# dfm/george

Measured on NVIDIA H100. Metric: gp.compute+log_likelihood N-points/sec, higher is better.
Workload: dtype f64

## Files before the change

george_b200/csrc/hodlr_leaf.cuh:

```cuda
#pragma once

#include "gemm_dmma.cuh"
#include "hodlr_kernels.cuh"

namespace bgp {

constexpr int LF_THREADS = 256;
constexpr int LF_NB = 32;
constexpr int LF_MAX_LEAF = 768;

__host__ __device__ inline int lf_panel_ld(int max_m) { return ((max_m + 15) / 16) * 16 + 4; }

template <int SHAPE>
__global__ void __launch_bounds__(LF_THREADS, 2) leaf_factor_kernel(const DevProgram* __restrict__ gprog,
                                                                    const double* __restrict__ x,
                                                                    const double* __restrict__ diag,
                                                                    const LeafDesc* __restrict__ leaves,
                                                                    double* __restrict__ Lbuf,
                                                                    double* __restrict__ leaf_logdet, int ldp) {
  extern __shared__ __align__(16) double lf_smem[];
  double* pn = lf_smem;
  double* dall = lf_smem + LF_NB * ldp;
  DevProgram* P = reinterpret_cast<DevProgram*>(lf_smem + (LF_NB + 1) * ldp);
  __shared__ double red[32];
  __shared__ double dinv[LF_NB];
  if constexpr (SHAPE == BGP_SHAPE_GENERIC) stage_program(P, gprog);
  __syncthreads();
  const auto fn = ShapeEval<SHAPE>::make(P, gprog);
  const LeafDesc lf = leaves[blockIdx.x];
  const int m = lf.size, nd = gprog->ndim;
  double* A = Lbuf + lf.off;
  const double* xs = x + (int64_t)lf.start * nd;
  const int lane = threadIdx.x & 31, warp = threadIdx.x >> 5;

  double logdet = 0.0;
  for (int k0 = 0; k0 < m; k0 += LF_NB) {
    const int nb = min(LF_NB, m - k0), rem = m - k0;
    for (int t = threadIdx.x; t < nb * rem; t += LF_THREADS) {
      const int c = t / rem, i = t - c * rem;
      if (i >= c) {
        double v = fn(xs + (int64_t)(k0 + i) * nd, xs + (int64_t)(k0 + c) * nd);
        if (i == c) v += diag[lf.start + k0 + i];
        pn[c * ldp + i] = v;
      }
    }
    __syncthreads();
    if (k0 > 0) {
      const int lr = lane >> 2, lc = lane & 3;
      const int n_tiles = (rem + 15) / 16;
      bool bok[4];
#pragma unroll
      for (int b = 0; b < 4; ++b) bok[b] = b * 8 + lr < nb;
      for (int t = warp; t < n_tiles; t += LF_THREADS / 32) {
        const int r0 = t * 16;
        bool aok[2];
#pragma unroll
        for (int a = 0; a < 2; ++a) aok[a] = r0 + a * 8 + lr < rem;
        double acc[2][4][2];
#pragma unroll
        for (int a = 0; a < 2; ++a)
#pragma unroll
          for (int b = 0; b < 4; ++b) { acc[a][b][0] = 0.0; acc[a][b][1] = 0.0; }
#pragma unroll 4
        for (int q0 = 0; q0 < k0; q0 += 4) {
          const int q = q0 + lc;
          const double* Lq = A + (int64_t)q * m + k0;
          const double dq = dall[q];
          double af[2], bf[4];
#pragma unroll
          for (int a = 0; a < 2; ++a) af[a] = aok[a] ? Lq[r0 + a * 8 + lr] : 0.0;
#pragma unroll
          for (int b = 0; b < 4; ++b) bf[b] = bok[b] ? Lq[b * 8 + lr] * dq : 0.0;
#pragma unroll
          for (int a = 0; a < 2; ++a)
#pragma unroll
            for (int b = 0; b < 4; ++b) dmma884(acc[a][b][0], acc[a][b][1], af[a], bf[b]);
        }
#pragma unroll
        for (int a = 0; a < 2; ++a) {
          const int i = r0 + a * 8 + lr;
#pragma unroll
          for (int b = 0; b < 4; ++b)
#pragma unroll
            for (int e = 0; e < 2; ++e) {
              const int c = b * 8 + 2 * lc + e;
              if (i < rem && c < nb && i >= c) pn[c * ldp + i] -= acc[a][b][e];
            }
        }
      }
      __syncthreads();
    }
    if (warp == 0) {
      double w[LF_NB];
#pragma unroll
      for (int j = 0; j < LF_NB; ++j) w[j] = (j <= lane && lane < nb) ? pn[j * ldp + lane] : 0.0;
#pragma unroll
      for (int k = 0; k < LF_NB; ++k) {
        if (k < nb) {
          const double d = __shfl_sync(0xffffffffu, w[k], k);
          const double l = (lane > k && lane < nb) ? w[k] / d : 0.0;
          if (lane > k) w[k] = l;
          const double ld = l * d;
#pragma unroll
          for (int j = k + 1; j < LF_NB; ++j) {
            const double lj = __shfl_sync(0xffffffffu, l, j);
            if (j <= lane) w[j] -= ld * lj;
          }
        }
      }
      if (lane < nb) {
        double* col = A + (int64_t)k0 * m + k0 + lane;
        double d = 0.0;
#pragma unroll
        for (int j = 0; j < LF_NB; ++j) {
          if (j < lane) { pn[j * ldp + lane] = w[j]; col[(int64_t)j * m] = w[j]; }
          if (j == lane) d = w[j];
        }
        col[(int64_t)lane * m] = d;
        dall[k0 + lane] = d;
        dinv[lane] = 1.0 / d;
        logdet += log(fabs(d));
      }
    }
    __syncthreads();
    const volatile double* l11 = pn;
    for (int i = LF_NB + threadIdx.x; i < rem; i += LF_THREADS) {
      double w[LF_NB];
#pragma unroll
      for (int j = 0; j < LF_NB; ++j) w[j] = pn[j * ldp + i];
#pragma unroll
      for (int j = 0; j < LF_NB; ++j) {
        double s = w[j];
#pragma unroll
        for (int q = 0; q < j; ++q) s -= w[q] * l11[q * ldp + j];
        w[j] = s;
      }
      double* row = A + (int64_t)k0 * m + k0 + i;
#pragma unroll
      for (int j = 0; j < LF_NB; ++j) row[(int64_t)j * m] = w[j] * dinv[j];
    }
    __syncthreads();
  }
  logdet = block_sum(logdet, red);
  if (threadIdx.x == 0) leaf_logdet[blockIdx.x] = logdet;
}

__host__ inline size_t lf_smem_bytes(int shape, int max_m) {
  return sizeof(double) * (size_t)(LF_NB + 1) * lf_panel_ld(max_m) + (shape == BGP_SHAPE_GENERIC ? sizeof(DevProgram) : 0);
}

template <int SHAPE>
inline void leaf_factor_launch_shape(int n_leaves, int max_m, cudaStream_t s, const DevProgram* prog, const double* x,
                                     const double* diag, const LeafDesc* leaves, double* L, double* leaf_logdet) {
  const size_t smem = lf_smem_bytes(SHAPE, max_m);
  cudaFuncSetAttribute(leaf_factor_kernel<SHAPE>, cudaFuncAttributeMaxDynamicSharedMemorySize, (int)smem);
  leaf_factor_kernel<SHAPE><<<n_leaves, LF_THREADS, smem, s>>>(prog, x, diag, leaves, L, leaf_logdet, lf_panel_ld(max_m));
}

inline void leaf_factor_launch(int shape, int n_leaves, int max_m, cudaStream_t s, const DevProgram* prog,
                               const double* x, const double* diag, const LeafDesc* leaves, double* L,
                               double* leaf_logdet) {
  BGP_SHAPE_SWITCH(shape, (leaf_factor_launch_shape<SHAPE>(n_leaves, max_m, s, prog, x, diag, leaves, L, leaf_logdet)));
}

}
```

Measured before the change: 21.53 million.

## Invert diagonal block and apply panel solve via DMMA in leaf factorization

Replaces the per-row scalar triangular solve for the below-diagonal panel with an explicit inverse of the unit-lower 32x32 diagonal block, computed by warp shuffles, followed by a DMMA tensor-core GEMM. It also rewrites the diagonal LDL factorization as a shifting-register loop using a shared column buffer, adds a 4-way ILP kernel evaluation for non-generic shapes, and raises the unroll on the trailing update. Optional clock64 phase timing instrumentation is added under a compile flag. The goal is to move the serial-heavy panel solve onto tensor cores. In exchange it adds static shared memory, which can affect occupancy, and an explicit inverse is numerically less stable than forward substitution.

Result: faster. 22.81 million, median of 6 (+5.9%).

```diff
diff --git a/george_b200/csrc/hodlr_leaf.cuh b/george_b200/csrc/hodlr_leaf.cuh
--- a/george_b200/csrc/hodlr_leaf.cuh
+++ b/george_b200/csrc/hodlr_leaf.cuh
@@ -8,8 +8,44 @@
 constexpr int LF_THREADS = 256;
 constexpr int LF_NB = 32;
 constexpr int LF_MAX_LEAF = 768;
-
-__host__ __device__ inline int lf_panel_ld(int max_m) { return ((max_m + 15) / 16) * 16 + 4; }
+constexpr int LF_LDT = LF_NB + 4;
+
+__host__ __device__ constexpr int lf_panel_ld(int max_m) { return ((max_m + 15) / 16) * 16 + 4; }
+static_assert((LF_THREADS / 32) * 4 == LF_NB, "step (3b) gives each warp four columns of L11^-1");
+
+#ifdef BGP_LF_PHASE_TIMING
+__device__ unsigned long long lf_phase_cycles[5];
+__device__ unsigned int lf_phase_ctas;
+__device__ inline void lf_phase_report(const long long* ph, long long t_begin) {
+  if (threadIdx.x != 0) return;
+  for (int p = 0; p < 4; ++p) atomicAdd(&lf_phase_cycles[p], (unsigned long long)ph[p]);
+  atomicAdd(&lf_phase_cycles[4], (unsigned long long)(clock64() - t_begin));
+  __threadfence();
+  if (atomicAdd(&lf_phase_ctas, 1u) == gridDim.x - 1) {
+    const double c = 1.0 / gridDim.x;
+    printf("leaf_factor cycles per CTA (%u CTAs): build %.0f update %.0f diagonal %.0f below %.0f total %.0f\n",
+           gridDim.x, lf_phase_cycles[0] * c, lf_phase_cycles[1] * c, lf_phase_cycles[2] * c, lf_phase_cycles[3] * c,
+           lf_phase_cycles[4] * c);
+    for (int p = 0; p < 5; ++p) lf_phase_cycles[p] = 0;
+    lf_phase_ctas = 0;
+  }
+}
+#define LF_TIMER_INIT                      \
+  long long lf_ph[4] = {0, 0, 0, 0};       \
+  const long long lf_t0 = clock64();       \
+  long long lf_t = lf_t0;
+#define LF_STAMP(p)                          \
+  if (threadIdx.x == 0) {                    \
+    const long long t1_ = clock64();         \
+    lf_ph[p] += t1_ - lf_t;                  \
+    lf_t = t1_;                              \
+  }
+#define LF_TIMER_REPORT lf_phase_report(lf_ph, lf_t0);
+#else
+#define LF_TIMER_INIT
+#define LF_STAMP(p)
+#define LF_TIMER_REPORT
+#endif
 
 template <int SHAPE>
 __global__ void __launch_bounds__(LF_THREADS, 2) leaf_factor_kernel(const DevProgram* __restrict__ gprog,
@@ -23,7 +59,8 @@
   double* dall = lf_smem + LF_NB * ldp;
   DevProgram* P = reinterpret_cast<DevProgram*>(lf_smem + (LF_NB + 1) * ldp);
   __shared__ double red[32];
-  __shared__ double dinv[LF_NB];
+  __shared__ __align__(16) double tm[LF_NB * LF_LDT];
+  __shared__ double colb[2 * LF_NB];
   if constexpr (SHAPE == BGP_SHAPE_GENERIC) stage_program(P, gprog);
   __syncthreads();
   const auto fn = ShapeEval<SHAPE>::make(P, gprog);
@@ -32,19 +69,31 @@
   double* A = Lbuf + lf.off;
   const double* xs = x + (int64_t)lf.start * nd;
   const int lane = threadIdx.x & 31, warp = threadIdx.x >> 5;
+  constexpr int ilp = SHAPE == BGP_SHAPE_GENERIC ? 1 : 4;
 
   double logdet = 0.0;
+  LF_TIMER_INIT
   for (int k0 = 0; k0 < m; k0 += LF_NB) {
     const int nb = min(LF_NB, m - k0), rem = m - k0;
-    for (int t = threadIdx.x; t < nb * rem; t += LF_THREADS) {
-      const int c = t / rem, i = t - c * rem;
-      if (i >= c) {
-        double v = fn(xs + (int64_t)(k0 + i) * nd, xs + (int64_t)(k0 + c) * nd);
-        if (i == c) v += diag[lf.start + k0 + i];
-        pn[c * ldp + i] = v;
+    const bool below = rem > LF_NB;
+    for (int t0 = threadIdx.x; t0 < nb * rem; t0 += LF_THREADS * ilp) {
+      double v[ilp];
+      int ci[ilp], ii[ilp];
+#pragma unroll
+      for (int u = 0; u < ilp; ++u) {
+        const int t = min(t0 + u * LF_THREADS, nb * rem - 1);
+        ci[u] = t / rem;
+        ii[u] = t - ci[u] * rem;
+        v[u] = fn(xs + (int64_t)(k0 + ii[u]) * nd, xs + (int64_t)(k0 + ci[u]) * nd);
+      }
+#pragma unroll
+      for (int u = 0; u < ilp; ++u) {
+        const int c = ci[u], i = ii[u];
+        if (t0 + u * LF_THREADS < nb * rem && i >= c) pn[c * ldp + i] = i == c ? v[u] + diag[lf.start + k0 + i] : v[u];
       }
     }
     __syncthreads();
+    LF_STAMP(0)
     if (k0 > 0) {
       const int lr = lane >> 2, lc = lane & 3;
       const int n_tiles = (rem + 15) / 16;
@@ -61,7 +110,7 @@
         for (int a = 0; a < 2; ++a)
 #pragma unroll
           for (int b = 0; b < 4; ++b) { acc[a][b][0] = 0.0; acc[a][b][1] = 0.0; }
-#pragma unroll 4
+#pragma unroll 8
         for (int q0 = 0; q0 < k0; q0 += 4) {
           const int q = q0 + lc;
           const double* Lq = A + (int64_t)q * m + k0;
@@ -89,65 +138,105 @@
         }
       }
       __syncthreads();
+      LF_STAMP(1)
     }
     if (warp == 0) {
+      const int i = lane;
       double w[LF_NB];
 #pragma unroll
-      for (int j = 0; j < LF_NB; ++j) w[j] = (j <= lane && lane < nb) ? pn[j * ldp + lane] : 0.0;
-#pragma unroll
-      for (int k = 0; k < LF_NB; ++k) {
-        if (k < nb) {
-          const double d = __shfl_sync(0xffffffffu, w[k], k);
-          const double l = (lane > k && lane < nb) ? w[k] / d : 0.0;
-          if (lane > k) w[k] = l;
-          const double ld = l * d;
-#pragma unroll
-          for (int j = k + 1; j < LF_NB; ++j) {
-            const double lj = __shfl_sync(0xffffffffu, l, j);
-            if (j <= lane) w[j] -= ld * lj;
+      for (int j = 0; j < LF_NB; ++j) w[j] = (j <= i && i < nb) ? pn[j * ldp + i] : 0.0;
+      double dmine = 1.0;
+      for (int k = 0; k < nb; ++k) {
+        double* cb = colb + (k & 1) * LF_NB;
+        cb[i] = w[0];
+        __syncwarp();
+        const double d = cb[k];
+        const bool act = i > k && i < nb;
+        const double l = act ? w[0] * (1.0 / d) : 0.0;
+        if (i == k) dmine = d;
+#pragma unroll
+        for (int j = 1; j < LF_NB; ++j) w[j - 1] = w[j] - l * cb[(k + j) & (LF_NB - 1)];
+        w[LF_NB - 1] = 0.0;
+        if (act) pn[k * ldp + i] = l;
+      }
+      if (i < nb) {
+        double* row = A + (int64_t)k0 * m + k0 + i;
+        for (int j = 0; j < i; ++j) row[(int64_t)j * m] = pn[j * ldp + i];
+        row[(int64_t)i * m] = dmine;
+        dall[k0 + i] = dmine;
+        logdet += log(fabs(dmine));
+      }
+    }
+    __syncthreads();
+    LF_STAMP(2)
+    if (below) {
+      const int i = lane;
+      const double rd = 1.0 / dall[k0 + i];
+      double mq[4];
+#pragma unroll
+      for (int c = 0; c < 4; ++c) mq[c] = i == 4 * warp + c ? 1.0 : 0.0;
+      for (int p = 0; p < LF_NB - 1; ++p) {
+        const double lip = i > p ? pn[p * ldp + i] : 0.0;
+#pragma unroll
+        for (int c = 0; c < 4; ++c) mq[c] -= lip * __shfl_sync(0xffffffffu, mq[c], p);
+      }
+#pragma unroll
+      for (int c = 0; c < 4; ++c) tm[(4 * warp + c) * LF_LDT + i] = mq[c] * rd;
+      __syncthreads();
+    }
+    if (below) {
+      const int lr = lane >> 2, lc = lane & 3;
+      const int n_tiles = (rem - LF_NB + 15) / 16;
+      for (int t = warp; t < n_tiles; t += LF_THREADS / 32) {
+        const int r0 = LF_NB + t * 16;
+        bool aok[2];
+#pragma unroll
+        for (int a = 0; a < 2; ++a) aok[a] = r0 + a * 8 + lr < rem;
+        double acc[2][4][2];
+#pragma unroll
+        for (int a = 0; a < 2; ++a)
+#pragma unroll
+          for (int b = 0; b < 4; ++b) { acc[a][b][0] = 0.0; acc[a][b][1] = 0.0; }
+#pragma unroll
+        for (int q0 = 0; q0 < LF_NB; q0 += 4) {
+          const int q = q0 + lc;
+          double af[2], bf[4];
+#pragma unroll
+          for (int a = 0; a < 2; ++a) af[a] = aok[a] ? pn[q * ldp + r0 + a * 8 + lr] : 0.0;
+#pragma unroll
+          for (int b = 0; b < 4; ++b) bf[b] = tm[q * LF_LDT + b * 8 + lr];
+#pragma unroll
+          for (int a = 0; a < 2; ++a)
+#pragma unroll
+            for (int b = 0; b < 4; ++b) dmma884(acc[a][b][0], acc[a][b][1], af[a], bf[b]);
+        }
+#pragma unroll
+        for (int a = 0; a < 2; ++a) {
+          const int i = r0 + a * 8 + lr;
+          if (i < rem) {
+            double* row = A + (int64_t)k0 * m + k0 + i;
+#pragma unroll
+            for (int b = 0; b < 4; ++b)
+#pragma unroll
+              for (int e = 0; e < 2; ++e) row[(int64_t)(b * 8 + 2 * lc + e) * m] = acc[a][b][e];
           }
         }
       }
-      if (lane < nb) {
-        double* col = A + (int64_t)k0 * m + k0 + lane;
-        double d = 0.0;
-#pragma unroll
-        for (int j = 0; j < LF_NB; ++j) {
-          if (j < lane) { pn[j * ldp + lane] = w[j]; col[(int64_t)j * m] = w[j]; }
-          if (j == lane) d = w[j];
-        }
-        col[(int64_t)lane * m] = d;
-        dall[k0 + lane] = d;
-        dinv[lane] = 1.0 / d;
-        logdet += log(fabs(d));
-      }
     }
     __syncthreads();
-    const volatile double* l11 = pn;
-    for (int i = LF_NB + threadIdx.x; i < rem; i += LF_THREADS) {
-      double w[LF_NB];
-#pragma unroll
-      for (int j = 0; j < LF_NB; ++j) w[j] = pn[j * ldp + i];
-#pragma unroll
-      for (int j = 0; j < LF_NB; ++j) {
-        double s = w[j];
-#pragma unroll
-        for (int q = 0; q < j; ++q) s -= w[q] * l11[q * ldp + j];
-        w[j] = s;
-      }
-      double* row = A + (int64_t)k0 * m + k0 + i;
-#pragma unroll
-      for (int j = 0; j < LF_NB; ++j) row[(int64_t)j * m] = w[j] * dinv[j];
-    }
-    __syncthreads();
+    LF_STAMP(3)
   }
+  LF_TIMER_REPORT
   logdet = block_sum(logdet, red);
   if (threadIdx.x == 0) leaf_logdet[blockIdx.x] = logdet;
 }
 
-__host__ inline size_t lf_smem_bytes(int shape, int max_m) {
+__host__ __device__ constexpr size_t lf_smem_bytes(int shape, int max_m) {
   return sizeof(double) * (size_t)(LF_NB + 1) * lf_panel_ld(max_m) + (shape == BGP_SHAPE_GENERIC ? sizeof(DevProgram) : 0);
 }
+constexpr size_t LF_STATIC_SMEM = sizeof(double) * (32 + LF_NB * LF_LDT + 2 * LF_NB);
+static_assert(lf_smem_bytes(BGP_SHAPE_GENERIC, LF_MAX_LEAF) + LF_STATIC_SMEM <= 232448,
+              "leaf_factor_kernel does not fit one SM's shared memory at LF_MAX_LEAF rows");
 
 template <int SHAPE>
 inline void leaf_factor_launch_shape(int n_leaves, int max_m, cudaStream_t s, const DevProgram* prog, const double* x,
```
